# szpiech/garlic

Hardware: AMD Instinct MI355X
Metric: LOD-windows/sec (SNPs x inds / winsize) (higher is better)
Workload: dtype f64

## Files before the change

### garlic_amd/csrc/garlic_hip.hip

```cpp
#include "../../include/garlic_hip.h"
#include "lod_kernels.hpp"
#include "variant_kernels.hpp"
#include "ld_kernels.hpp"
#include "ld_multi_kernel.hpp"
#include "tgls_ring_kernel.hpp"
#include "tgls_feed_kernel.hpp"
#include "tgls_feed_multi_kernel.hpp"
#include "wlod_strip_kernel.hpp"
#include "wlod_small_kernel.hpp"
#include "coverage_kernel.hpp"
#include "roh_segments_kernel.hpp"
#include "feed_kernel.hpp"
#include "wlod_feed_kernel.hpp"

#include <algorithm>
#include <chrono>
#include <functional>
#include <memory>
#include <mutex>
#include <queue>
#include <cmath>
#include <cstdarg>
#include <cstdio>
#include <cstdlib>
// ... 2267 lines not shown
        hipError_t e = hipSuccess;
        if (where == GARLIC_HOST) {
            if ((rc = stage.reserve((size_t)(rows * ld)))) { stage.release(); return rc; }
            e = hipMemcpyAsync(stage.p, src, (size_t)(rows * ld), hipMemcpyHostToDevice, s);
            src = stage.p;
        }
        if (e == hipSuccess) {
            const int64_t waves = rows * nblk;
            hipLaunchKernelGGL(phase_planes_kernel, dim3((unsigned)((waves + 3) / 4)), dim3(256), 0, s, src,
                               ld, locus_begin + done, rows, p->nind, nblk, p->nloci, p->d_phase.p);
            e = hipGetLastError();
        }
        if (e == hipSuccess) e = hipStreamSynchronize(s);
        if (e != hipSuccess) { stage.release(); return fail(GARLIC_ERR_HIP, "set_phase: %s", hipGetErrorString(e)); }
    }
    stage.release();
    p->have_phase = true;
    return GARLIC_OK;
}

static int reserve_skew_buf(garlic_panel *p, DevBuf<double> &buf, int32_t winsize, bool zero)
{
    int rc;
    const size_t nskew = SKEW_FRONT + ((size_t)p->nloci + winsize + 64) * winsize;
    if ((rc = buf.reserve(nskew))) return rc;
    if (zero) {
        HIP_TRY(hipMemsetAsync(buf.p, 0, sizeof(double) * nskew, p->ctx->stream));
    } else {
        HIP_TRY(hipMemsetAsync(buf.p, 0, sizeof(double) * SKEW_FRONT, p->ctx->stream));
        const size_t body = SKEW_FRONT + (size_t)p->nloci * winsize;
        HIP_TRY(hipMemsetAsync(buf.p + body, 0, sizeof(double) * (nskew - body), p->ctx->stream));
    }
    return GARLIC_OK;
}
static int reserve_skew(garlic_panel *p, int32_t winsize, bool zero = true)
{
    return reserve_skew_buf(p, p->d_skew, winsize, zero);
}

static void drop_ld_sets(garlic_panel *p) { p->ld_sets.clear(); }
static bool select_ld(garlic_panel *p, int32_t winsize)
{
    if (p->have_ld && p->ld_winsize == winsize) return true;
    for (size_t i = 0; i < p->ld_sets.size(); i++) {
        garlic_panel::LdSet &set = *p->ld_sets[i];
        if (set.W != winsize) continue;
        std::swap(set.skew.p, p->d_skew.p);
        std::swap(set.skew.cap, p->d_skew.cap);
        std::swap(set.group, p->ld_group);
        if (p->have_ld) set.W = p->ld_winsize;
        else p->ld_sets.erase(p->ld_sets.begin() + (ptrdiff_t)i);
        p->ld_winsize = winsize;
        p->have_ld = true;
        p->rld_valid = false;
        return true;
    }
    return false;
}
static void stash_ld(garlic_panel *p, int32_t group)
{
    if (!p->have_ld) return;
    std::unique_ptr<garlic_panel::LdSet> set(new garlic_panel::LdSet);
    set->W = p->ld_winsize;
    set->group = group;
    std::swap(set->skew.p, p->d_skew.p);
    std::swap(set->skew.cap, p->d_skew.cap);
    p->ld_sets.push_back(std::move(set));
    p->have_ld = false;
    p->rld_valid = false;
    p->ld_winsize = 0;
    p->ld_group = -1;
}
static void drop_all_ld(garlic_panel *p)
{
    drop_ld_sets(p);
    p->d_skew.release();
    p->d_rld.release();
    p->have_ld = p->rld_valid = false;
    p->ld_winsize = 0;
    p->ld_group = -1;
}

static int install_ld(garlic_panel *p, int32_t winsize, const double *src, bool skew_done = false)
{
    int rc;
    hipStream_t s = p->ctx->stream;
    if (!skew_done) {
        if ((rc = reserve_skew(p, winsize))) return rc;
        for (int c = 0; c < p->nchr; c++)
            hipLaunchKernelGGL(skew_reciprocal_kernel, dim3(1024), dim3(256), 0, s, src,
                               p->d_skew.p + SKEW_FRONT, p->chr_off[c], p->chr_off[c + 1], winsize);
    }
    HIP_TRY(hipGetLastError());
    HIP_TRY(hipStreamSynchronize(s));
    p->d_rld.release();
    p->rld_valid = false;
    p->have_ld = true;
    p->ld_winsize = winsize;
    p->ld_group = -1;
    if (!p->ld_multi_active) {
        drop_ld_sets(p);
        p->ld_pair_passes = p->ld_sum_passes = 0;
    }
    return GARLIC_OK;
}

static int ensure_rld(garlic_panel *p)
{
    if (p->rld_valid) return GARLIC_OK;
    int rc;
    const int32_t W = p->ld_winsize;
    if ((rc = p->d_rld.reserve((size_t)p->nloci * W))) return rc;
    for (int c = 0; c < p->nchr; c++)
        hipLaunchKernelGGL(unskew_kernel, dim3(1024), dim3(256), 0, p->ctx->stream, p->d_skew.p + SKEW_FRONT, p->d_rld.p,
                           p->chr_off[c], p->chr_off[c + 1], W);
    HIP_TRY(hipGetLastError());
    p->rld_valid = true;
    return GARLIC_OK;
}

int garlic_panel_set_ld(garlic_panel *p, int32_t winsize, const double *ld, int32_t where)
{
    if (!p || !ld) return fail(GARLIC_ERR_INVALID, "panel and ld are required");
    if (winsize <= 1) return fail(GARLIC_ERR_INVALID, "winsize must be > 1");
    int rc;
    if ((rc = set_device(p->ctx))) return rc;
    const size_t n = (size_t)p->nloci * winsize;
    const double *src = ld;
    if (where == GARLIC_HOST) {
        if ((rc = p->d_stage64.reserve(n))) return rc;
        HIP_TRY(hipMemcpyAsync(p->d_stage64.p, ld, sizeof(double) * n, hipMemcpyHostToDevice,
                               p->ctx->stream));
        src = p->d_stage64.p;
    }
    rc = install_ld(p, winsize, src);
    p->d_stage64.release();
    return rc;
}

static bool ld_pairs_on_mfma(int32_t winsize, int32_t phased)
{
    const int mfma_nj = 1 + (30 + winsize) / 32;
    const bool pair_flat = getenv("GARLIC_LD_PAIR_FLAT") && winsize <= 32;
    return !phased && !pair_flat && winsize > LD_SMALL_MAX_W && mfma_nj <= 5 && !getenv("GARLIC_LD_PAIR_NO_MFMA") &&
           !getenv("GARLIC_LD_PAIR_TILED") && !getenv("GARLIC_LD_PAIR_L2");
}
static bool ld_sums_by_snp(int32_t winsize)
{
    const int col_threads = (winsize + 16 + WAVE - 1) / WAVE * WAVE;
    return winsize > LD_COL_B && winsize <= 512 && col_threads <= LD_COL_MAX_THREADS && !getenv("GARLIC_LD_SUM_BY_COLUMN") &&
           !getenv("GARLIC_LD_SUM_L2");
}

static int ld_check(garlic_panel *p, int32_t winsize, int32_t phased)
{
    if (!p) return fail(GARLIC_ERR_INVALID, "panel is NULL");
    if (!p->have_geno) return fail(GARLIC_ERR_STATE, "panel needs genotypes before LD weights");
    if (phased && !p->have_phase)
        return fail(GARLIC_ERR_STATE, "phased LD weights need garlic_panel_set_phase first");
    if (phased && !p->have_freq)
        return fail(GARLIC_ERR_STATE, "phased LD weights need the allele frequencies (garlic_panel_set_freq)");
    if (winsize <= 1) return fail(GARLIC_ERR_INVALID, "winsize must be > 1");
    if ((int64_t)p->nloci * winsize * 2 >= ((int64_t)1 << 40))
        return fail(GARLIC_ERR_INVALID, "LD table of %lld x %d too large", (long long)p->nloci, winsize);
    return set_device(p->ctx);
}

int garlic_ld_counts(garlic_panel *p, int32_t winsize, int32_t phased, const int32_t *sub_idx, int32_t n_sub,
                     int32_t *locus_counts, int32_t *pair_counts, int32_t where)
{
    int rc;
    if ((rc = ld_check(p, winsize, phased))) return rc;
    if (!locus_counts || !pair_counts) return fail(GARLIC_ERR_INVALID, "count buffers are required");
    if (n_sub < 0 || (n_sub > 0 && !sub_idx)) return fail(GARLIC_ERR_INVALID, "bad LD subsample");
    hipStream_t s = p->ctx->stream;
    const int nblk = (int)(p->nind_pad / WAVE);
    std::vector<uint64_t> sub((size_t)nblk, 0);
    if (!sub_idx) {
        for (int i = 0; i < p->nind; i++) sub[i >> 6] |= (uint64_t)1 << (i & 63);
    } else {
        for (int k = 0; k < n_sub; k++) {
            const int i = sub_idx[k];
            if (i < 0 || i >= p->nind)
                return fail(GARLIC_ERR_INVALID, "LD subsample index %d outside panel of %d", i, p->nind);
            if (sub[i >> 6] & ((uint64_t)1 << (i & 63)))
                return fail(GARLIC_ERR_INVALID, "LD subsample index %d given twice", i);
            sub[i >> 6] |= (uint64_t)1 << (i & 63);
        }
    }
    DevBuf<uint64_t> &d_sub = p->lds.sub, &d_m = p->lds.m, &d_h = p->lds.h, &d_o = p->lds.o;
    DevBuf<int32_t> &d_loc = p->lds.loc, &d_pair = p->lds.pair;
    const size_t npl = (size_t)nblk * p->nloci, npair = (size_t)p->nloci * winsize * 2;
    if ((rc = d_sub.reserve(nblk)) || (rc = d_m.reserve(npl)) || (rc = d_h.reserve(npl))) return rc;
    if (phased && (rc = d_o.reserve(npl))) return rc;
    int32_t *loc = locus_counts, *pair = pair_counts;
    if (where == GARLIC_HOST) {
        if ((rc = d_loc.reserve((size_t)p->nloci * 2)) || (rc = d_pair.reserve(npair))) return rc;
        loc = d_loc.p; pair = d_pair.p;
    }
    const bool pair_flat = getenv("GARLIC_LD_PAIR_FLAT") && winsize <= 32;
    const int lane_stage = std::min(nblk, getenv("GARLIC_LD_LANE_STAGE") ? atoi(getenv("GARLIC_LD_LANE_STAGE")) : 4);
    const int lane_dc = winsize - 1 <= 16 ? 16 : 32;
    const size_t lane_lds = sizeof(uint64_t) * (phased ? 4 : 2) * (size_t)lane_stage * (LD_LANE_T + winsize - 1);
    const int mfma_nj = 1 + (30 + winsize) / 32;
    const bool pair_mfma = ld_pairs_on_mfma(winsize, phased);
    const bool fuse_hr2 = p->lds.fuse_request && pair_mfma && ld_sums_by_snp(winsize);
    if (p->lds.fuse_request && !fuse_hr2) {
        p->lds.fuse_request = false;
        return fail(GARLIC_ERR_STATE, "internal: LD fusion requested for a shape the pair kernel does not take");
    }
    p->lds.fuse_request = false;
    p->lds.fused_done = false;
    const bool pair_lane = !pair_mfma && !pair_flat && winsize - 1 <= 256 && lane_lds <= 150 * 1024 && !getenv("GARLIC_LD_PAIR_TILED") &&
                           !getenv("GARLIC_LD_PAIR_L2");
    const bool pair_tiled = !pair_mfma && !pair_flat && !pair_lane && winsize - 1 <= 256 && !getenv("GARLIC_LD_PAIR_L2");
    hipError_t e = hipMemcpyAsync(d_sub.p, sub.data(), sizeof(uint64_t) * nblk, hipMemcpyHostToDevice, s);
    if (e == hipSuccess && !pair_tiled && !pair_flat && !pair_lane && !pair_mfma) e = hipMemsetAsync(pair, 0, sizeof(int32_t) * npair, s);
    if (e != hipSuccess) return fail(GARLIC_ERR_HIP, "LD counts: %s", hipGetErrorString(e));
    uint64_t planes_key = 0xCBF29CE484222325ull;
    for (uint64_t w : sub) planes_key = (planes_key ^ w) * 0x100000001B3ull;
    planes_key = (planes_key ^ (uint64_t)(phased ? 2 : 1)) * 0x100000001B3ull;
    planes_key = (planes_key ^ p->geno_epoch) * 0x100000001B3ull;
    planes_key = (planes_key ^ (uint64_t)nblk) * 0x100000001B3ull;
    if ((rc = p->lds.loc_planes.reserve((size_t)p->nloci * 2))) return rc;
    if (!(p->lds.planes_valid && p->lds.planes_key == planes_key) || getenv("GARLIC_LD_NO_PLANE_CACHE")) {
        p->lds.planes_valid = false;
        if (phased)
            hipLaunchKernelGGL(ld_planes_kernel<true>, dim3((unsigned)p->nwordrows), dim3(256), 0, s, p->d_packed.p,
                               p->nwordrows, nblk, d_sub.p, p->nloci, d_m.p, d_h.p, d_o.p, p->lds.loc_planes.p);
        else
            hipLaunchKernelGGL(ld_planes_kernel<false>, dim3((unsigned)p->nwordrows), dim3(256), 0, s, p->d_packed.p,
                               p->nwordrows, nblk, d_sub.p, p->nloci, d_m.p, d_h.p, (uint64_t *)nullptr, p->lds.loc_planes.p);
        e = hipGetLastError();
        if (e != hipSuccess) return fail(GARLIC_ERR_HIP, "LD planes: %s", hipGetErrorString(e));
        p->lds.planes_key = planes_key;
        p->lds.planes_valid = true;
    }
    e = hipMemcpyAsync(loc, p->lds.loc_planes.p, sizeof(int32_t) * p->nloci * 2, hipMemcpyDeviceToDevice, s);
    if (e != hipSuccess) return fail(GARLIC_ERR_HIP, "LD counts: %s", hipGetErrorString(e));
    const int pair_threads = (winsize - 1 + WAVE - 1) / WAVE * WAVE;
    const size_t pair_lds = sizeof(uint64_t) * (phased ? 4 : 2) * LD_PAIR_BLK * (LD_PAIR_T + winsize - 1);
    if (pair_tiled && pair_lds > 48 * 1024) {
        const void *fn = phased ? (const void *)ld_pair_tiled_kernel<true> : (const void *)ld_pair_tiled_kernel<false>;
        hipError_t ae = hipFuncSetAttribute(fn, hipFuncAttributeMaxDynamicSharedMemorySize, (int)pair_lds);
        if (ae != hipSuccess) return fail(GARLIC_ERR_HIP, "LD counts: %s", hipGetErrorString(ae));
    }
    if (pair_tiled) {
        std::vector<LdPairChr> pc;
        int64_t blocks = 0;
        for (int c = 0; c < p->nchr; c++) {
            pc.push_back(LdPairChr{p->chr_off[c], p->chr_off[c + 1], blocks});
            blocks += (p->chr_nloci[c] + LD_PAIR_T - 1) / LD_PAIR_T;
        }
        DevBuf<LdPairChr> &d_pc = p->lds.pair_chrs;
        if ((rc = d_pc.reserve(pc.size()))) return rc;
        e = hipMemcpyAsync(d_pc.p, pc.data(), sizeof(LdPairChr) * pc.size(), hipMemcpyHostToDevice, s);
        if (e != hipSuccess) return fail(GARLIC_ERR_HIP, "LD counts: %s", hipGetErrorString(e));
        if (phased)
            hipLaunchKernelGGL(ld_pair_tiled_kernel<true>, dim3((unsigned)blocks), dim3(pair_threads), pair_lds, s, d_m.p,
                               d_h.p, d_o.p, p->d_phase.p, nblk, p->nloci, d_pc.p, p->nchr, winsize, pair);
        else
            hipLaunchKernelGGL(ld_pair_tiled_kernel<false>, dim3((unsigned)blocks), dim3(pair_threads), pair_lds, s, d_m.p,
                               d_h.p, (const uint64_t *)nullptr, (const uint64_t *)nullptr, nblk, p->nloci, d_pc.p,
                               p->nchr, winsize, pair);
        e = hipGetLastError();
        if (e == hipSuccess) e = hipStreamSynchronize(s);
        if (e != hipSuccess) return fail(GARLIC_ERR_HIP, "LD counts: %s", hipGetErrorString(e));
    }
    if (pair_mfma) {
        std::vector<LdPairChr> pc;
        int64_t blocks = 0;
        for (int c = 0; c < p->nchr; c++) {
            pc.push_back(LdPairChr{p->chr_off[c], p->chr_off[c + 1], blocks});
            blocks += (p->chr_nloci[c] + LDM_TI - 1) / LDM_TI;
        }
        DevBuf<LdPairChr> &d_pc = p->lds.pair_chrs;
        if ((rc = d_pc.reserve(pc.size()))) return rc;
        e = hipMemcpyAsync(d_pc.p, pc.data(), sizeof(LdPairChr) * pc.size(), hipMemcpyHostToDevice, s);
        const void *fn = fuse_hr2 ? (mfma_nj <= 2 ? (const void *)ld_pair_mfma_kernel<2, true> : mfma_nj == 3 ? (const void *)ld_pair_mfma_kernel<3, true>
                                     : mfma_nj == 4 ? (const void *)ld_pair_mfma_kernel<4, true> : (const void *)ld_pair_mfma_kernel<5, true>)
                                  : (mfma_nj <= 2 ? (const void *)ld_pair_mfma_kernel<2, false> : mfma_nj == 3 ? (const void *)ld_pair_mfma_kernel<3, false>
                                     : mfma_nj == 4 ? (const void *)ld_pair_mfma_kernel<4, false> : (const void *)ld_pair_mfma_kernel<5, false>);
        const int nj = std::max(2, mfma_nj);
        const size_t lds = std::max((size_t)2 * 2 * (4 + nj - 1) * WAVE * 16, fuse_hr2 ? LDM_XT_BYTES : (size_t)0);
        const double *a_hf = nullptr;
        double *a_c = nullptr;
        if (fuse_hr2) {
            const size_t n = (size_t)p->nloci * winsize;
            if ((rc = p->lds.hf.reserve(p->nloci)) || (rc = p->lds.fwd.reserve(2 * n + 256))) return rc;
            hipLaunchKernelGGL(ld_homfreq_kernel, dim3((unsigned)((p->nloci + 255) / 256)), dim3(256), 0, s, p->lds.loc_planes.p, p->nloci,
                               p->lds.hf.p);
            a_hf = p->lds.hf.p;
            a_c = p->lds.fwd.p;
        }
        if (e == hipSuccess && lds > 48 * 1024) e = hipFuncSetAttribute(fn, hipFuncAttributeMaxDynamicSharedMemorySize, (int)lds);
        if (e != hipSuccess) return fail(GARLIC_ERR_HIP, "LD counts: %s", hipGetErrorString(e));
        const uint64_t *a_m = d_m.p, *a_h = d_h.p;
        const LdPairChr *a_pc = d_pc.p;
        int a_nblk = nblk, a_nchr = p->nchr, a_w = winsize;
        int64_t a_nloci = p->nloci;
        void *kargs[] = {(void *)&a_m, (void *)&a_h, (void *)&a_nblk, (void *)&a_nloci, (void *)&a_pc, (void *)&a_nchr, (void *)&a_w, (void *)&pair,
                         (void *)&a_hf, (void *)&a_c};
        e = hipLaunchKernel(fn, dim3((unsigned)blocks), dim3(256), kargs, lds, s);
        if (e == hipSuccess) e = hipStreamSynchronize(s);
        if (e != hipSuccess) return fail(GARLIC_ERR_HIP, "LD counts: %s", hipGetErrorString(e));
        p->lds.fused_done = fuse_hr2;
    }
    if (pair_lane) {
        std::vector<LdPairChr> pc;
        int64_t blocks = 0;
        for (int c = 0; c < p->nchr; c++) {
            pc.push_back(LdPairChr{p->chr_off[c], p->chr_off[c + 1], blocks});
            blocks += (p->chr_nloci[c] + LD_LANE_T - 1) / LD_LANE_T;
        }
        DevBuf<LdPairChr> &d_pc = p->lds.pair_chrs;
        if ((rc = d_pc.reserve(pc.size()))) return rc;
        e = hipMemcpyAsync(d_pc.p, pc.data(), sizeof(LdPairChr) * pc.size(), hipMemcpyHostToDevice, s);
        const void *fn = lane_dc == 16 ? (phased ? (const void *)ld_pair_lane_kernel<true, 16> : (const void *)ld_pair_lane_kernel<false, 16>)
                                       : (phased ? (const void *)ld_pair_lane_kernel<true, 32> : (const void *)ld_pair_lane_kernel<false, 32>);
        if (e == hipSuccess && lane_lds > 48 * 1024) e = hipFuncSetAttribute(fn, hipFuncAttributeMaxDynamicSharedMemorySize, (int)lane_lds);
        if (e != hipSuccess) return fail(GARLIC_ERR_HIP, "LD counts: %s", hipGetErrorString(e));
        const uint64_t *a_m = d_m.p, *a_h = d_h.p, *a_o = phased ? d_o.p : nullptr, *a_f = phased ? p->d_phase.p : nullptr;
        const LdPairChr *a_pc = d_pc.p;
        int a_nblk = nblk, a_nchr = p->nchr, a_w = winsize, a_stage = lane_stage;
        int64_t a_nloci = p->nloci;
        void *kargs[] = {(void *)&a_m, (void *)&a_h, (void *)&a_o, (void *)&a_f, (void *)&a_nblk, (void *)&a_nloci, (void *)&a_pc,
                         (void *)&a_nchr, (void *)&a_w, (void *)&a_stage, (void *)&pair};
        e = hipLaunchKernel(fn, dim3((unsigned)blocks), dim3(LD_LANE_T), kargs, lane_lds, s);
        if (e == hipSuccess) e = hipStreamSynchronize(s);
        if (e != hipSuccess) return fail(GARLIC_ERR_HIP, "LD counts: %s", hipGetErrorString(e));
    }
    if (pair_flat) {
        const unsigned grid = (unsigned)(((int64_t)p->nloci * winsize + 255) / 256);
        if (phased)
            hipLaunchKernelGGL(ld_pair_flat_kernel<true>, dim3(grid), dim3(256), 0, s, d_m.p, d_h.p, d_o.p, p->d_phase.p, nblk,
                               p->nloci, p->d_chr_off.p, p->nchr, winsize, pair);
        else
            hipLaunchKernelGGL(ld_pair_flat_kernel<false>, dim3(grid), dim3(256), 0, s, d_m.p, d_h.p, (const uint64_t *)nullptr,
                               (const uint64_t *)nullptr, nblk, p->nloci, p->d_chr_off.p, p->nchr, winsize, pair);
    }
    for (int c = 0; !pair_tiled && !pair_flat && !pair_lane && !pair_mfma && c < p->nchr; c++) {
        if (phased)
            hipLaunchKernelGGL(ld_pair_phased_kernel, dim3((unsigned)p->chr_nloci[c]), dim3(256), 0, s, d_m.p,
                               d_h.p, d_o.p, p->d_phase.p, nblk, p->nloci, p->chr_off[c], p->chr_off[c + 1],
                               winsize, pair);
        else
            hipLaunchKernelGGL(ld_pair_kernel, dim3((unsigned)p->chr_nloci[c]), dim3(256), 0, s, d_m.p, d_h.p,
                               nblk, p->nloci, p->chr_off[c], p->chr_off[c + 1], winsize, pair);
    }
    e = hipGetLastError();
    if (e == hipSuccess && where == GARLIC_HOST) {
        e = hipMemcpyAsync(locus_counts, loc, sizeof(int32_t) * p->nloci * 2, hipMemcpyDeviceToHost, s);
        if (e == hipSuccess)
            e = hipMemcpyAsync(pair_counts, pair, sizeof(int32_t) * npair, hipMemcpyDeviceToHost, s);
    }
    if (e == hipSuccess) e = hipStreamSynchronize(s);
    if (e != hipSuccess) return fail(GARLIC_ERR_HIP, "LD counts: %s", hipGetErrorString(e));
    return GARLIC_OK;
}

int garlic_ld_finish(garlic_panel *p, int32_t winsize, int32_t phased, const int32_t *locus_counts,
                     const int32_t *pair_counts, double *ld_out, int32_t where)
{
    int rc;
    if ((rc = ld_check(p, winsize, phased))) return rc;
    if (!locus_counts || !pair_counts) return fail(GARLIC_ERR_INVALID, "count buffers are required");
    hipStream_t s = p->ctx->stream;
    const size_t n = (size_t)p->nloci * winsize;
    DevBuf<int32_t> &d_loc = p->lds.loc, &d_pair = p->lds.pair;
    DevBuf<double> &d_hf = p->lds.hf, &d_fwd = p->lds.fwd, &d_bwd = p->lds.bwd, &d_ld = p->lds.ld;
    DevBuf<LdSumChr> &d_sum_chrs = p->lds.sum_chrs;
    const int32_t *loc = locus_counts, *pair = pair_counts;
    hipError_t e = hipSuccess;
    if (where == GARLIC_HOST) {
        if ((rc = d_loc.reserve((size_t)p->nloci * 2)) || (rc = d_pair.reserve(n * 2))) return rc;
        e = hipMemcpyAsync(d_loc.p, locus_counts, sizeof(int32_t) * p->nloci * 2, hipMemcpyHostToDevice, s);
        if (e == hipSuccess)
            e = hipMemcpyAsync(d_pair.p, pair_counts, sizeof(int32_t) * n * 2, hipMemcpyHostToDevice, s);
        loc = d_loc.p; pair = d_pair.p;
    }
    if (winsize <= LD_SMALL_MAX_W && !getenv("GARLIC_LD_NO_FLAT")) {
        if ((rc = d_hf.reserve(p->nloci))) return rc;
        double *ld = ld_out;
        if (where == GARLIC_HOST || !ld_out) {
            if ((rc = d_ld.reserve(n))) return rc;
            ld = d_ld.p;
        }
        if (e == hipSuccess) e = hipMemsetAsync(ld, 0, sizeof(double) * n, s);
        if (e == hipSuccess && phased) e = hipMemcpyAsync(d_hf.p, p->freq.data(), sizeof(double) * p->nloci, hipMemcpyHostToDevice, s);
        if (e != hipSuccess) return fail(GARLIC_ERR_HIP, "LD finish: %s", hipGetErrorString(e));
        if (!phased)
            hipLaunchKernelGGL(ld_homfreq_kernel, dim3((unsigned)((p->nloci + 255) / 256)), dim3(256), 0, s, loc, p->nloci, d_hf.p);
        garlic_ctx *ctx = p->ctx;
        const int slot = (int)(ctx->n_calls % garlic_ctx::HIST);
        (void)hipEventRecord(ctx->hist0[slot], s);
        hipLaunchKernelGGL(ld_sum_flat_kernel, dim3((unsigned)((n + 255) / 256)), dim3(256), 0, s, pair, d_hf.p, p->d_chr_off.p,
                           p->nchr, p->nloci, winsize, ld);
        (void)hipEventRecord(ctx->hist1[slot], s);
        ctx->n_calls++;
        e = hipGetLastError();
        if (e != hipSuccess) return fail(GARLIC_ERR_HIP, "LD finish: %s", hipGetErrorString(e));
        if ((rc = install_ld(p, winsize, ld, false))) return rc;
        if (where == GARLIC_HOST && ld_out) {
            e = hipMemcpyAsync(ld_out, ld, sizeof(double) * n, hipMemcpyDeviceToHost, s);
            if (e == hipSuccess) e = hipStreamSynchronize(s);
            if (e != hipSuccess) return fail(GARLIC_ERR_HIP, "LD finish: %s", hipGetErrorString(e));
        }
        return GARLIC_OK;
    }
    const int col_threads = (winsize + 16 + WAVE - 1) / WAVE * WAVE;
    const bool by_snp = ld_sums_by_snp(winsize);
    const bool have_table = p->lds.fused_done && by_snp;
    p->lds.fused_done = false;
    const bool tiled = by_snp || (winsize <= LD_SUM_MAX_W && !getenv("GARLIC_LD_SUM_L2"));
    const int sum_b = by_snp ? std::min(LD_COL_B, col_threads - winsize) : LD_SUM_B;
    if ((rc = d_hf.reserve(p->nloci)) || (rc = d_fwd.reserve(by_snp ? 2 * n + 256 : n)) || (!by_snp && (rc = d_bwd.reserve(n))))
        return rc;
    double *ld = ld_out;
    const bool weights_only = by_snp && !ld_out;
    if (!weights_only && (where == GARLIC_HOST || !ld_out)) {
        if ((rc = d_ld.reserve(n))) return rc;
        ld = d_ld.p;
    }
    if (weights_only) {
    } else if (by_snp) {
        for (int c = 0; c < p->nchr && e == hipSuccess; c++) {
            const int64_t lo = p->chr_off[c], hi = p->chr_off[c + 1], from = std::max(lo, hi - winsize + 1);
            if (hi > from) e = hipMemsetAsync(ld + from * winsize, 0, sizeof(double) * (size_t)(hi - from) * winsize, s);
        }
    } else {
        e = hipMemsetAsync(ld, 0, sizeof(double) * n, s);
    }
    if (e != hipSuccess) return fail(GARLIC_ERR_HIP, "LD finish: %s", hipGetErrorString(e));
    if (phased) {
        e = hipMemcpyAsync(d_hf.p, p->freq.data(), sizeof(double) * p->nloci, hipMemcpyHostToDevice, s);
        if (e != hipSuccess) return fail(GARLIC_ERR_HIP, "LD finish: %s", hipGetErrorString(e));
    } else {
        hipLaunchKernelGGL(ld_homfreq_kernel, dim3((unsigned)((p->nloci + 255) / 256)), dim3(256), 0, s, loc,
                           p->nloci, d_hf.p);
    }
    std::vector<LdSumChr> sum_chrs;
    int64_t sum_blocks = 0;
    for (int c = 0; tiled && c < p->nchr; c++) {
        const int64_t nstarts = p->chr_off[c + 1] - p->chr_off[c] - winsize + 1;
        if (nstarts < 1) continue;
        sum_chrs.push_back(LdSumChr{p->chr_off[c], nstarts, sum_blocks});
        sum_blocks += (nstarts + sum_b - 1) / sum_b;
    }
    if (tiled && (rc = d_sum_chrs.reserve(std::max<size_t>(sum_chrs.size(), 1)))) return rc;
    if (by_snp && (rc = reserve_skew(p, winsize, false))) return rc;
    for (int c = 0; c < p->nchr; c++) {
        const int64_t lo = p->chr_off[c], hi = p->chr_off[c + 1];
        const size_t hr2_lds = sizeof(double) * (LD_HR2_T + winsize + (size_t)LD_HR2_T * (winsize + 1));
        if (have_table)
            ;
        else if (by_snp && hr2_lds <= 64 * 1024 && !getenv("GARLIC_LD_HR2_PLAIN"))
            hipLaunchKernelGGL(ld_hr2_tile_kernel, dim3((unsigned)((hi - lo + LD_HR2_T - 1) / LD_HR2_T)), dim3(256),
                               hr2_lds, s, pair, d_hf.p, lo, hi, winsize, d_fwd.p);
        else if (by_snp)
            hipLaunchKernelGGL(ld_hr2_kernel<true>, dim3((unsigned)(hi - lo)), dim3(128), 0, s, pair, d_hf.p, lo, hi,
                               winsize, d_fwd.p, (double *)nullptr);
        else
            hipLaunchKernelGGL(ld_hr2_kernel<false>, dim3((unsigned)(hi - lo)), dim3(256), 0, s, pair, d_hf.p, lo, hi,
                               winsize, d_fwd.p, d_bwd.p);
        if (hi - lo >= winsize && !tiled)
            hipLaunchKernelGGL(ld_sum_kernel, dim3((unsigned)(hi - lo - winsize + 1)), dim3(256), 0, s, d_fwd.p, d_bwd.p,
                               lo, winsize, ld);
    }
    if (tiled && !sum_chrs.empty()) {
        e = hipMemcpyAsync(d_sum_chrs.p, sum_chrs.data(), sizeof(LdSumChr) * sum_chrs.size(), hipMemcpyHostToDevice, s);
        if (e != hipSuccess) return fail(GARLIC_ERR_HIP, "LD finish: %s", hipGetErrorString(e));
        const int threads = by_snp ? col_threads : (winsize + WAVE - 1) / WAVE * WAVE;
        const int col_pieces = (threads * 8 + 1023) / 1024;
        const size_t lds = by_snp ? sizeof(double) * std::max<size_t>((size_t)LD_COL_BATCH * LD_COL_NBATCH * col_pieces * 128 + 130, (size_t)threads * 17)
                                  : sizeof(double) * 2 * (2 * (size_t)winsize - 1 + 128 + threads);
        garlic_ctx *ctx = p->ctx;
        const int slot = (int)(ctx->n_calls % garlic_ctx::HIST);
        (void)hipEventRecord(ctx->hist0[slot], s);
        if (by_snp) {
            static_assert(LD_COL_MAX_THREADS <= 128 * LD_COL_MAX_PIECES, "one instantiation per request count");
            const void *fn = col_pieces == 1 ? (const void *)ld_sum_col_kernel<1> : col_pieces == 2 ? (const void *)ld_sum_col_kernel<2>
                           : col_pieces == 3 ? (const void *)ld_sum_col_kernel<3> : col_pieces == 4 ? (const void *)ld_sum_col_kernel<4>
                                                                                                    : (const void *)ld_sum_col_kernel<5>;
            if (lds > 48 * 1024) {
                e = hipFuncSetAttribute(fn, hipFuncAttributeMaxDynamicSharedMemorySize, (int)lds);
                if (e != hipSuccess) return fail(GARLIC_ERR_HIP, "LD finish: %s", hipGetErrorString(e));
            }
            const double *a_c = d_fwd.p;
            const LdSumChr *a_chrs = d_sum_chrs.p;
            int a_nchr = (int)sum_chrs.size(), a_w = winsize, a_b = sum_b;
            double *a_ld = ld, *a_d = p->d_skew.p + SKEW_FRONT;
            unsigned a_nwork = (unsigned)sum_blocks;
            void *kargs[] = {(void *)&a_c, (void *)&a_chrs, (void *)&a_nchr, (void *)&a_w, (void *)&a_b, (void *)&a_ld, (void *)&a_d, (void *)&a_nwork};
            e = hipLaunchKernel(fn, dim3((a_nwork + 7u) / 8u * 8u), dim3(threads), kargs, lds, s);
            if (e != hipSuccess) return fail(GARLIC_ERR_HIP, "LD finish: %s", hipGetErrorString(e));
        }
        else
            hipLaunchKernelGGL(ld_sum_tiled_kernel, dim3((unsigned)sum_blocks), dim3(threads), lds, s, d_fwd.p, d_bwd.p,
                               d_sum_chrs.p, (int)sum_chrs.size(), winsize, ld);
        (void)hipEventRecord(ctx->hist1[slot], s);
        ctx->n_calls++;
    }
    e = hipGetLastError();
    if (e != hipSuccess) return fail(GARLIC_ERR_HIP, "LD finish: %s", hipGetErrorString(e));
    if ((rc = install_ld(p, winsize, ld, by_snp))) return rc;
    if (where == GARLIC_HOST && ld_out) {
        e = hipMemcpyAsync(ld_out, ld, sizeof(double) * n, hipMemcpyDeviceToHost, s);
        if (e == hipSuccess) e = hipStreamSynchronize(s);
        if (e != hipSuccess) return fail(GARLIC_ERR_HIP, "LD finish: %s", hipGetErrorString(e));
    }
    return GARLIC_OK;
}

int garlic_panel_compute_ld(garlic_panel *p, int32_t winsize, int32_t phased, const int32_t *sub_idx,
                            int32_t n_sub, double *ld_out, int32_t where)
{
    int rc;
    if ((rc = ld_check(p, winsize, phased))) return rc;
    DevBuf<int32_t> &d_loc = p->lds.loc, &d_pair = p->lds.pair;
    const bool fuse = ld_pairs_on_mfma(winsize, phased) && ld_sums_by_snp(winsize) && !getenv("GARLIC_LD_UNFUSED");
    if ((rc = d_loc.reserve((size_t)p->nloci * 2)) || (rc = d_pair.reserve(fuse ? 2 : (size_t)p->nloci * winsize * 2)))
        return rc;
    p->lds.fuse_request = fuse;
    if ((rc = garlic_ld_counts(p, winsize, phased, sub_idx, n_sub, d_loc.p, d_pair.p, GARLIC_DEVICE))) {
        p->lds.fuse_request = false;
        return rc;
    }
    if (where == GARLIC_DEVICE || !ld_out)
        return garlic_ld_finish(p, winsize, phased, d_loc.p, d_pair.p, ld_out, GARLIC_DEVICE);
    DevBuf<double> &d_ld = p->lds.ld;
    if ((rc = d_ld.reserve((size_t)p->nloci * winsize))) return rc;
    rc = garlic_ld_finish(p, winsize, phased, d_loc.p, d_pair.p, d_ld.p, GARLIC_DEVICE);
    if (rc == GARLIC_OK) {
        hipError_t e = hipMemcpy(ld_out, d_ld.p, sizeof(double) * p->nloci * winsize, hipMemcpyDeviceToHost);
        if (e != hipSuccess) rc = fail(GARLIC_ERR_HIP, "LD copy-out: %s", hipGetErrorString(e));
    }
    return rc;
}

static int ld_col_threads(int32_t winsize) { return (winsize + 16 + WAVE - 1) / WAVE * WAVE; }

struct LdMultiPlan {
    std::vector<int32_t> uniq;
    std::vector<std::vector<int32_t>> groups;
    size_t n_shared = 0;
    int32_t wtab = 0;
};
static LdMultiPlan ld_multi_plan(const int32_t *winsizes, int32_t n_sizes)
{
    LdMultiPlan plan;
    plan.uniq.assign(winsizes, winsizes + n_sizes);
    std::sort(plan.uniq.begin(), plan.uniq.end());
    plan.uniq.erase(std::unique(plan.uniq.begin(), plan.uniq.end()), plan.uniq.end());
    const char *solo_env = getenv("GARLIC_LD_MULTI_SOLO");
    const bool solo = solo_env && atoi(solo_env) != 0;
    std::vector<int32_t> sharing, alone;
    for (int32_t w : plan.uniq) (!solo && ld_sums_by_snp(w) ? sharing : alone).push_back(w);
    if (sharing.size() < 2) {
        alone = plan.uniq;
        sharing.clear();
    }
    for (int32_t w : sharing) {
        const bool fits = !plan.groups.empty() && plan.groups.back().size() < (size_t)LDM_MAX_SIZES &&
                          ldms_lds_bytes(ld_col_threads(w), (int)plan.groups.back().size()) <= LDMS_LDS_MAX;
        if (!fits) plan.groups.emplace_back();
        plan.groups.back().push_back(w);
    }
    plan.n_shared = plan.groups.size();
    plan.wtab = sharing.empty() ? 0 : sharing.back();
    for (int32_t w : alone) plan.groups.push_back(std::vector<int32_t>{w});
    return plan;
}

typedef std::vector<std::unique_ptr<garlic_panel::LdSet>> LdSetPool;
static std::unique_ptr<garlic_panel::LdSet> ld_pool_take(LdSetPool &pool, int32_t winsize)
{
    for (size_t i = 0; i < pool.size(); i++)
        if (pool[i]->W == winsize) {
            std::unique_ptr<garlic_panel::LdSet> set = std::move(pool[i]);
            pool.erase(pool.begin() + (ptrdiff_t)i);
            return set;
        }
    std::unique_ptr<garlic_panel::LdSet> set(new garlic_panel::LdSet);
    set->W = winsize;
    return set;
}

static int ld_build_table(garlic_panel *p, int32_t W, int32_t phased, const int32_t *loc, const int32_t *pair)
{
    int rc;
    hipStream_t s = p->ctx->stream;
    const size_t n = (size_t)p->nloci * W;
    if ((rc = p->lds.hf.reserve(p->nloci)) || (rc = p->lds.fwd.reserve(2 * n + 256))) return rc;
    if (phased)
        HIP_TRY(hipMemcpyAsync(p->lds.hf.p, p->freq.data(), sizeof(double) * p->nloci, hipMemcpyHostToDevice, s));
    else
        hipLaunchKernelGGL(ld_homfreq_kernel, dim3((unsigned)((p->nloci + 255) / 256)), dim3(256), 0, s, loc, p->nloci, p->lds.hf.p);
    const size_t hr2_lds = sizeof(double) * (LD_HR2_T + W + (size_t)LD_HR2_T * (W + 1));
    for (int c = 0; c < p->nchr; c++) {
        const int64_t lo = p->chr_off[c], hi = p->chr_off[c + 1];
        if (hr2_lds <= 64 * 1024 && !getenv("GARLIC_LD_HR2_PLAIN"))
            hipLaunchKernelGGL(ld_hr2_tile_kernel, dim3((unsigned)((hi - lo + LD_HR2_T - 1) / LD_HR2_T)), dim3(256), hr2_lds, s, pair,
                               p->lds.hf.p, lo, hi, W, p->lds.fwd.p);
        else
            hipLaunchKernelGGL(ld_hr2_kernel<true>, dim3((unsigned)(hi - lo)), dim3(128), 0, s, pair, p->lds.hf.p, lo, hi, W,
                               p->lds.fwd.p, (double *)nullptr);
    }
    HIP_TRY(hipGetLastError());
    return GARLIC_OK;
}

static int ld_multi_group(garlic_panel *p, const std::vector<int32_t> &g, int32_t gid, int32_t wtab, double *const *dev_ld,
                          LdSetPool &pool)
{
    int rc;
    hipStream_t s = p->ctx->stream;
    const int32_t W = g.back(), wmin = g.front();
    const int threads = ld_col_threads(W), B = std::min(LD_COL_B, threads - W), pieces = (threads * 8 + 1023) / 1024;
    const size_t lds = ldms_lds_bytes(threads, (int)g.size() - 1);
    std::vector<LdMultiChr> chrs;
    int64_t blocks = 0;
    for (int c = 0; c < p->nchr; c++) {
        const int64_t lo = p->chr_off[c], hi = p->chr_off[c + 1], nstarts = hi - lo - wmin + 1;
        if (nstarts < 1) continue;
        chrs.push_back(LdMultiChr{lo, hi, nstarts, blocks});
        blocks += (nstarts + B - 1) / B;
    }
    std::vector<std::unique_ptr<garlic_panel::LdSet>> sets;
    LdMultiSmall small{};
    small.n = (int32_t)g.size() - 1;
    for (size_t i = 0; i < g.size(); i++) {
        sets.push_back(ld_pool_take(pool, g[i]));
// ... 1457 lines not shown
```

### garlic_amd/csrc/ld_kernels.hpp

```cpp
#pragma once
#include "lod_kernels.hpp"
#include "tgls_math.hpp"
#include "variant_kernels.hpp"

namespace garlic {

__device__ __forceinline__ double x86_nan_if_nan(double v)
{
    return v != v ? f64_from_bits(X86_DEFAULT_NAN) : v;
}

__device__ __forceinline__ uint32_t ld_writelane(uint32_t v, int lane, uint32_t old)
{
    asm("v_writelane_b32 %0, %1, %2" : "+v"(old) : "s"(v), "n"(lane));
    return old;
}

template <bool PHASED>
__global__ void __launch_bounds__(256)
ld_planes_kernel(const uint32_t *__restrict__ packed, int64_t nwordrows, int nblk,
                 const uint64_t *__restrict__ submask, int64_t nloci, uint64_t *__restrict__ planeM,
                 uint64_t *__restrict__ planeH, uint64_t *__restrict__ planeO, int32_t *__restrict__ counts)
{
    __shared__ int32_t red[4][16][2];
// ... 566 lines not shown
        LD_COL_WAIT_CASE(57)
        LD_COL_WAIT_CASE(58)
        LD_COL_WAIT_CASE(59)
        LD_COL_WAIT_CASE(60)
        LD_COL_WAIT_CASE(61)
        LD_COL_WAIT_CASE(62)
        LD_COL_WAIT_CASE(63)
#undef LD_COL_WAIT_CASE
    default: asm volatile("s_waitcnt vmcnt(0)" ::: "memory"); break;
    }
}

#define LD_COL_ADD(q) "v_add_f64 %[a" #q "], %[a" #q "], %[h]\n\t"
#define LD_COL_OPS(a)                                                                                              \
    [a0] "+v"(a[0]), [a1] "+v"(a[1]), [a2] "+v"(a[2]), [a3] "+v"(a[3]), [a4] "+v"(a[4]), [a5] "+v"(a[5]),          \
    [a6] "+v"(a[6]), [a7] "+v"(a[7]), [a8] "+v"(a[8]), [a9] "+v"(a[9]), [a10] "+v"(a[10]), [a11] "+v"(a[11]),      \
    [a12] "+v"(a[12]), [a13] "+v"(a[13]), [a14] "+v"(a[14]), [a15] "+v"(a[15]), [a16] "+v"(a[16]),                 \
    [a17] "+v"(a[17]), [a18] "+v"(a[18]), [a19] "+v"(a[19]), [a20] "+v"(a[20]), [a21] "+v"(a[21]),                 \
    [a22] "+v"(a[22]), [a23] "+v"(a[23]), [a24] "+v"(a[24]), [a25] "+v"(a[25]), [a26] "+v"(a[26]),                 \
    [a27] "+v"(a[27]), [a28] "+v"(a[28]), [a29] "+v"(a[29]), [a30] "+v"(a[30]), [a31] "+v"(a[31])
#define LD_COL_JUMP "s_getpc_b64 s[98:99]\n\ts_add_u32 s98, s98, %[off]\n\ts_addc_u32 s99, s99, 0\n\ts_setpc_b64 s[98:99]\n\t"
__device__ __forceinline__ void ld_col_adds(double (&a)[LD_COL_B], double h, bool ascending, int first)
{
    static_assert(LD_COL_B == 32, "32 adds are written out");
    const uint32_t off = (uint32_t)__builtin_amdgcn_readfirstlane(first * 8 + (ascending ? 12 + 32 * 8 + 4 : 12));
    asm volatile(LD_COL_JUMP
                 LD_COL_ADD(31) LD_COL_ADD(30) LD_COL_ADD(29) LD_COL_ADD(28) LD_COL_ADD(27) LD_COL_ADD(26)
                 LD_COL_ADD(25) LD_COL_ADD(24) LD_COL_ADD(23) LD_COL_ADD(22) LD_COL_ADD(21) LD_COL_ADD(20)
                 LD_COL_ADD(19) LD_COL_ADD(18) LD_COL_ADD(17) LD_COL_ADD(16) LD_COL_ADD(15) LD_COL_ADD(14)
                 LD_COL_ADD(13) LD_COL_ADD(12) LD_COL_ADD(11) LD_COL_ADD(10) LD_COL_ADD(9) LD_COL_ADD(8) LD_COL_ADD(7)
                 LD_COL_ADD(6) LD_COL_ADD(5) LD_COL_ADD(4) LD_COL_ADD(3) LD_COL_ADD(2) LD_COL_ADD(1) LD_COL_ADD(0)
                 "s_branch LD_COL_END_%=\n\t"
                 LD_COL_ADD(0) LD_COL_ADD(1) LD_COL_ADD(2) LD_COL_ADD(3) LD_COL_ADD(4) LD_COL_ADD(5)
                 LD_COL_ADD(6) LD_COL_ADD(7) LD_COL_ADD(8) LD_COL_ADD(9) LD_COL_ADD(10) LD_COL_ADD(11) LD_COL_ADD(12)
                 LD_COL_ADD(13) LD_COL_ADD(14) LD_COL_ADD(15) LD_COL_ADD(16) LD_COL_ADD(17) LD_COL_ADD(18)
                 LD_COL_ADD(19) LD_COL_ADD(20) LD_COL_ADD(21) LD_COL_ADD(22) LD_COL_ADD(23) LD_COL_ADD(24)
                 LD_COL_ADD(25) LD_COL_ADD(26) LD_COL_ADD(27) LD_COL_ADD(28) LD_COL_ADD(29) LD_COL_ADD(30)
                 LD_COL_ADD(31)
                 "LD_COL_END_%=:\n\t"
                 : LD_COL_OPS(a) : [h] "v"(h), [off] "s"(off) : "s98", "s99", "scc");
}
template <int PIECES>
__global__ void __launch_bounds__(LD_COL_MAX_THREADS)
ld_sum_col_kernel(const double *__restrict__ C, const LdSumChr *__restrict__ chrs, int nchr, int W, int B,
                  double *__restrict__ ld, double *__restrict__ D, unsigned nwork)
{
    const unsigned per_xcd = gridDim.x >> 3;
    const unsigned vblock = (blockIdx.x & 7u) * per_xcd + (blockIdx.x >> 3);
    if (vblock >= nwork) return;
    constexpr int BATCH = LD_COL_BATCH, NB = LD_COL_NBATCH, NRING = BATCH * NB, STEADY = (NB - 2) * BATCH * PIECES;
    static_assert(STEADY <= 63, "requests that can be counted");
    extern __shared__ double ld_rows[];
    const int tl = threadIdx.x, P = 2 * W;
    const int wave = __builtin_amdgcn_readfirstlane(threadIdx.x >> 6);
    int c = 0;
    while (c + 1 < nchr && (int64_t)vblock >= chrs[c + 1].block0) c++;
    const int64_t s0 = chrs[c].lo + ((int64_t)vblock - chrs[c].block0) * B;
    const int ns = (int)min<int64_t>(B, chrs[c].lo + chrs[c].nstarts - s0);
    const int nsteps = ns + W - 1, nbatches = (nsteps + BATCH - 1) / BATCH;
    const uint32_t ring = (uint32_t)(uintptr_t)(__attribute__((address_space(3))) double *)ld_rows;
    constexpr uint32_t row_bytes = (uint32_t)PIECES * 1024u, ring_bytes = row_bytes * NRING;
    const uint32_t lane16 = (uint32_t)(tl & 63) * 16u;
    const char *req_row = reinterpret_cast<const char *>(C + s0 * P);
    int req_e = W - 1, req_left = nsteps;
    uint32_t req_off = 0;
    auto request_batch = [&]() {
#pragma unroll
        for (int u = 0; u < BATCH; u++) {
            if (req_left > 0) {
                const char *g = req_row + (int64_t)(req_e & ~1) * 8;
#pragma unroll
                for (int q = 0; q < PIECES; q++)
                    asm volatile("s_mov_b32 m0, %0\n\ts_nop 0\n\tglobal_load_lds_dwordx4 %1, %2"
                                 :: "s"(ring + req_off + (uint32_t)q * 1024u), "v"(lane16), "s"(g + q * 1024) : "memory");
                req_row += (int64_t)P * 8;
                req_e--;
                req_left--;
            }
            req_off += row_bytes;
        }
        if (req_off == ring_bytes) req_off = 0;
    };
    if (wave == 0)
        for (int k = 0; k < NB - 1; k++) request_batch();
    double acc[LD_COL_B];
#pragma unroll
    for (int q = 0; q < LD_COL_B; q++) acc[q] = 0.0;
    uint32_t rd_addr = ring + (uint32_t)tl * 8u;
    const uint32_t rd_end = rd_addr + ring_bytes;
    uint32_t odd = (uint32_t)(W - 1) & 1u;
    static_assert(BATCH % 2 == 0, "the parity of W-1-j repeats per batch");
    for (int k = 0; k < nbatches; k++) {
        if (wave == 0) {
            const int rows_later = min(nsteps, (k + NB - 1) * BATCH) - (k + 1) * BATCH;
            if (rows_later == (NB - 2) * BATCH) asm volatile("s_waitcnt vmcnt(%0)" ::"n"(STEADY) : "memory");
            else ld_col_wait(max(rows_later, 0) * PIECES);
        }
        __syncthreads();
        if (wave == 0) request_batch();
        const int j0 = k * BATCH;
        double h[BATCH];
#pragma unroll
        for (int u = 0; u < BATCH; u++)
            asm volatile("ds_read_b64 %0, %1" : "=v"(h[u]) : "v"(rd_addr + (uint32_t)u * row_bytes + ((odd ^ (uint32_t)(u & 1)) * 8u)) : "memory");
        asm volatile("s_waitcnt lgkmcnt(0)" ::: "memory");
        rd_addr += BATCH * row_bytes;
        if (rd_addr == rd_end) rd_addr -= ring_bytes;
#pragma unroll
        for (int u = 0; u < BATCH; u++) {
            const int j = j0 + u;
#ifdef GARLIC_LDS_ABL_NO_ADDS
            if (j < nsteps && h[u] == 1.2345e-300) {
#else
            if (j < nsteps) {
#endif
                const bool leaving = j >= W;
                ld_col_adds(acc, h[u], leaving,
                            leaving ? j - W + 1 : (j < LD_COL_B - 1 ? LD_COL_B - 1 - j : 0));
            }
        }
    }
#ifndef GARLIC_LDS_ABL_NO_LD
    if (ld) {
#pragma unroll
        for (int q = 0; q < LD_COL_B; q++) {
            const int k = tl - q;
            if (q < ns && k >= 0 && k < W) ld[(s0 + q) * W + k] = x86_nan_if_nan(acc[q]);
        }
    }
#else
    if (acc[0] == 1.2345e-300) ld[s0 * W + tl] = acc[1] + acc[2] + acc[3] + acc[31] + acc[16];
#endif
#ifdef GARLIC_LDS_ABL_NO_D
    if (acc[5] != 1.2345e-300) return;
#endif
    if (!D) return;
    __syncthreads();
    double *tile = ld_rows;
    const int nthreads = blockDim.x;
    for (int q0 = 0; q0 < LD_COL_B; q0 += 16) {
#pragma unroll
        for (int u = 0; u < 16; u++)
            if (q0 == 0) tile[tl * 17 + u] = reciprocal_x86(x86_nan_if_nan(acc[u]));
            else tile[tl * 17 + u] = reciprocal_x86(x86_nan_if_nan(acc[16 + u]));
        __syncthreads();
        for (int e = tl; e < nthreads * 16; e += nthreads) {
            const int t2 = e >> 4, u = e & 15, q = q0 + u, k = t2 - q;
            if (q < ns && k >= 0 && k < W) D[(s0 + t2) * W + k] = tile[t2 * 17 + u];
        }
        __syncthreads();
    }
}

}

namespace garlic {

constexpr int LDM_TI = 128;
typedef int ldm_i32x4 __attribute__((ext_vector_type(4)));

typedef int ldm_i32x8 __attribute__((ext_vector_type(8)));
typedef float ldm_f32x16 __attribute__((ext_vector_type(16)));

__device__ __forceinline__ uint32_t ldm_spread8(uint32_t x)
{
    uint32_t t = (x | (x << 12)) & 0x000F000Fu;
    t = (t | (t << 6)) & 0x03030303u;
    return (t | (t << 3)) & 0x11111111u;
}

constexpr int LDM_XT = 33;
constexpr size_t LDM_XT_BYTES = ((size_t)4 * 32 * LDM_XT + 256) * 8;

template <int NJ, bool HR2>
__global__ void __launch_bounds__(256, 2)
ld_pair_mfma_kernel(const uint64_t *__restrict__ planeM, const uint64_t *__restrict__ planeH, int nblk, int64_t nloci,
                    const LdPairChr *__restrict__ chrs, int nchr, int W, int32_t *__restrict__ pair,
                    const double *__restrict__ hf, double *__restrict__ C)
{
    constexpr int NT = 4 + NJ - 1;
    static_assert(NT * 32 <= 256, "one staged SNP per thread");
    constexpr int BUF = 2 * NT * WAVE * 16;
    extern __shared__ __attribute__((aligned(16))) unsigned char ldm_lds[];
    const int tid = threadIdx.x, lane = tid & 63;
    const int wave = __builtin_amdgcn_readfirstlane(tid >> 6);
    int c = 0;
    while (c + 1 < nchr && (int64_t)blockIdx.x >= chrs[c + 1].block0) c++;
    const int64_t hi = chrs[c].hi;
    const int64_t i0 = chrs[c].lo + ((int64_t)blockIdx.x - chrs[c].block0) * LDM_TI;
    const bool mine = tid < NT * 32;
    const bool in = mine && i0 + tid < hi;
    uint64_t wm = 0, wh = 0;
    auto fetch = [&](int b) {
        const int64_t g = (int64_t)b * nloci + i0 + (in ? tid : 0);
        wm = in ? planeM[g] : 0;
        wh = in ? planeH[g] : 0;
    };
    auto stage = [&](int buf) {
        if (!mine) return;
        const int tile = tid >> 5, r = tid & 31;
#pragma unroll
        for (int pl = 0; pl < 2; pl++) {
            const uint64_t w = pl ? wh : wm;
#pragma unroll
            for (int h = 0; h < 2; h++) {
                const uint32_t x = (uint32_t)(w >> (32 * h));
                unsigned char *dst = ldm_lds + buf * BUF + (((pl * NT + tile) * WAVE) + h * 32 + r) * 16;
                *reinterpret_cast<uint4 *>(dst) = make_uint4(ldm_spread8(x & 0xFFu), ldm_spread8((x >> 8) & 0xFFu),
                                                             ldm_spread8((x >> 16) & 0xFFu), ldm_spread8(x >> 24));
            }
        }
    };
    ldm_f32x16 acc[NJ][2];
#pragma unroll
    for (int q = 0; q < NJ; q++)
#pragma unroll
        for (int pl = 0; pl < 2; pl++)
#pragma unroll
            for (int k = 0; k < 16; k++) acc[q][pl][k] = 0.0f;
    fetch(0);
    stage(0);
    if (nblk > 1) fetch(1);
    __syncthreads();
    const int one = 0x7F7F7F7F;
    for (int b = 0; b < nblk; b++) {
        const int buf = b & 1;
#ifndef GARLIC_LDM_ABL_NO_STAGE
        if (b + 1 < nblk) stage(buf ^ 1);
#endif
        if (b + 2 < nblk) fetch(b + 2);
#pragma unroll
        for (int pl = 0; pl < 2; pl++) {
            ldm_i32x8 fb[NJ];
#pragma unroll
            for (int q = 0; q < NJ; q++) {
                const ldm_i32x4 f = *reinterpret_cast<const ldm_i32x4 *>(ldm_lds + buf * BUF + (((pl * NT + wave + q) * WAVE) + lane) * 16);
                fb[q] = ldm_i32x8{f[0], f[1], f[2], f[3], 0, 0, 0, 0};
            }
#pragma unroll
            for (int q = 0; q < NJ; q++)
                acc[q][pl] = __builtin_amdgcn_mfma_scale_f32_32x32x64_f8f6f4(fb[0], fb[q], acc[q][pl], 4, 4, 0, one, 0, one);
        }
        __syncthreads();
    }
    const int col = lane & 31, rh = 4 * (lane >> 5);
    const int64_t it = i0 + wave * 32;
    if (HR2) {
        double *xt = reinterpret_cast<double *>(ldm_lds) + (size_t)wave * 32 * LDM_XT;
        double *hfs = reinterpret_cast<double *>(ldm_lds) + (size_t)4 * 32 * LDM_XT;
        if (mine) hfs[tid] = in ? hf[i0 + tid] : 0.0;
        __syncthreads();
        const int P = 2 * W;
#pragma unroll
        for (int q = 0; q < NJ; q++) {
            const int64_t j = it + q * 32 + col;
            const double HB = hfs[wave * 32 + q * 32 + col];
            const bool okB = HB > 0 && HB < 1;
            const double pB = HB * (1 - HB);
#pragma unroll
            for (int k = 0; k < 16; k++) {
                const int base = (k & 3) + 8 * (k >> 2);
                if (32 * q + 31 - base < 0 || 32 * q - (base + 4) >= W) continue;
                const int il = base + rh;
                const int64_t i = it + il;
                const int64_t d = j - i;
                const double HA = hfs[wave * 32 + il];
                double f = 0.0, b = 0.0;
                if (HA > 0 && HA < 1 && okB) {
                    double HAB = (double)(int)(acc[q][1][k] * 4.0f);
                    HAB /= (double)(int)(acc[q][0][k] * 4.0f);
                    const double H = HAB - HA * HB, HH = H * H;
                    const double vf = HH / (HA * (1 - HA) * HB * (1 - HB));
                    const double vb = HH / (pB * HA * (1 - HA));
                    f = (vf > 1) ? 1.0 : x86_nan_if_nan(vf);
                    b = (vb > 1) ? 1.0 : x86_nan_if_nan(vb);
                }
                if (i < hi && j < hi && d >= 0 && d < W) C[i * P + W - 1 + d] = d == 0 ? 1.0 : f;
                xt[col * LDM_XT + il] = b;
                __builtin_amdgcn_sched_barrier(0);
            }
            __builtin_amdgcn_fence(__ATOMIC_ACQ_REL, "wavefront");
#pragma unroll 4
            for (int r = 0; r < 16; r++) {
                const int jl = 2 * r + (lane >> 5);
                const int64_t jj = it + q * 32 + jl, ii = it + col;
                const int64_t d = jj - ii;
                const double v = xt[jl * LDM_XT + col];
                if (ii < hi && jj < hi && d >= 1 && d < W) C[jj * P + W - 1 - d] = v;
            }
            __builtin_amdgcn_fence(__ATOMIC_ACQ_REL, "wavefront");
        }
        return;
    }
#pragma unroll
    for (int q = 0; q < NJ; q++) {
        const int64_t j = it + q * 32 + col;
#pragma unroll
        for (int k = 0; k < 16; k++) {
            const int64_t i = it + (k & 3) + 8 * (k >> 2) + rh;
            const int64_t d = j - i;
            if (i < hi && d >= 0 && d < W) {
                int2 v = make_int2((int)(acc[q][0][k] * 4.0f), (int)(acc[q][1][k] * 4.0f));
                if (d == 0) v = make_int2(0, 0);
#ifdef GARLIC_LDM_ABL_NO_STORE
                if (v.x != 0x7FFFFFF1) continue;
#endif
// ... 8 lines not shown
```

Before: 7.193 billion.

## Add streaming LD column-sum kernel with async global-to-LDS ring buffer

Adds ld_sum_stream_kernel, which gives each block a span of K column batches. A dedicated loader wave streams the forward LD rows into an LDS ring buffer using global_load_lds_dwordx4 while G teams of threads consume successive batches in turn. The intent is to reuse overlapping window rows across adjacent batches within a block instead of reloading them per batch, and to overlap global loads with the accumulation. It also writes the reciprocal table through per-wave LDS tiles using only wave barriers. The cost is more complex scheduling, large LDS use, fewer blocks, and possible load imbalance depending on the span heuristic.

```diff
diff --git a/garlic_amd/csrc/garlic_hip.hip b/garlic_amd/csrc/garlic_hip.hip
--- a/garlic_amd/csrc/garlic_hip.hip
+++ b/garlic_amd/csrc/garlic_hip.hip
@@ -2443,6 +2443,33 @@
            !getenv("GARLIC_LD_SUM_L2");
 }
 
+struct LdStreamPlan {
+    bool ok;
+    int T, B, G, K, threads, loader_wave;
+    size_t lds;
+};
+static LdStreamPlan ld_sum_stream_plan(int32_t winsize, int64_t nloci)
+{
+    LdStreamPlan pl{};
+    if (!ld_sums_by_snp(winsize) || getenv("GARLIC_LD_SUM_NO_STREAM")) return pl;
+    pl.T = (winsize + 16 + WAVE - 1) / WAVE * WAVE;
+    pl.B = std::min(LD_COL_B, pl.T - winsize);
+    pl.G = (pl.B + winsize - 1 + pl.B - 1) / pl.B;
+    pl.lds = ld_stream_lds_bytes(winsize, pl.T);
+    if (pl.G * pl.T > LD_STREAM_MAX_THREADS || pl.lds > LD_STREAM_LDS_MAX) return pl;
+    const bool own_wave = pl.G * pl.T + WAVE <= LD_STREAM_MAX_THREADS;
+    pl.threads = pl.G * pl.T + (own_wave ? WAVE : 0);
+    pl.loader_wave = own_wave ? pl.G * pl.T / WAVE : 0;
+    int k = (int)std::ceil((winsize - 1) / (0.055 * pl.B));
+    const int64_t even = nloci / pl.B / 2048;
+    if (even < k) k = (int)std::max<int64_t>(even, pl.G);
+    if (const char *v = getenv("GARLIC_LD_STREAM_SPAN")) k = atoi(v);
+    else k = (k + pl.G - 1) / pl.G * pl.G;
+    pl.K = std::min(std::max(k, 1), LD_STREAM_MAX_SPAN);
+    pl.ok = true;
+    return pl;
+}
+
 static int ld_check(garlic_panel *p, int32_t winsize, int32_t phased)
 {
     if (!p) return fail(GARLIC_ERR_INVALID, "panel is NULL");
@@ -2730,13 +2757,15 @@
         hipLaunchKernelGGL(ld_homfreq_kernel, dim3((unsigned)((p->nloci + 255) / 256)), dim3(256), 0, s, loc,
                            p->nloci, d_hf.p);
     }
+    const LdStreamPlan stream = by_snp ? ld_sum_stream_plan(winsize, p->nloci) : LdStreamPlan{};
+    const int64_t sum_unit = stream.ok ? (int64_t)stream.K * sum_b : sum_b;
     std::vector<LdSumChr> sum_chrs;
     int64_t sum_blocks = 0;
     for (int c = 0; tiled && c < p->nchr; c++) {
         const int64_t nstarts = p->chr_off[c + 1] - p->chr_off[c] - winsize + 1;
         if (nstarts < 1) continue;
         sum_chrs.push_back(LdSumChr{p->chr_off[c], nstarts, sum_blocks});
-        sum_blocks += (nstarts + sum_b - 1) / sum_b;
+        sum_blocks += (nstarts + sum_unit - 1) / sum_unit;
     }
     if (tiled && (rc = d_sum_chrs.reserve(std::max<size_t>(sum_chrs.size(), 1)))) return rc;
     if (by_snp && (rc = reserve_skew(p, winsize, false))) return rc;
@@ -2768,7 +2797,18 @@
         garlic_ctx *ctx = p->ctx;
         const int slot = (int)(ctx->n_calls % garlic_ctx::HIST);
         (void)hipEventRecord(ctx->hist0[slot], s);
-        if (by_snp) {
+        if (stream.ok) {
+            const void *fn = (const void *)ld_sum_stream_kernel;
+            if (stream.lds > 48 * 1024) {
+                e = hipFuncSetAttribute(fn, hipFuncAttributeMaxDynamicSharedMemorySize, (int)stream.lds);
+                if (e != hipSuccess) return fail(GARLIC_ERR_HIP, "LD finish: %s", hipGetErrorString(e));
+            }
+            const unsigned nwork = (unsigned)sum_blocks;
+            hipLaunchKernelGGL(ld_sum_stream_kernel, dim3((nwork + 7u) / 8u * 8u), dim3((unsigned)stream.threads), stream.lds, s,
+                               (const double *)d_fwd.p, (const LdSumChr *)d_sum_chrs.p, (int)sum_chrs.size(), (int)winsize, stream.B,
+                               stream.G, stream.T, stream.K, stream.loader_wave, ld, p->d_skew.p + SKEW_FRONT, nwork);
+        }
+        else if (by_snp) {
             static_assert(LD_COL_MAX_THREADS <= 128 * LD_COL_MAX_PIECES, "one instantiation per request count");
             const void *fn = col_pieces == 1 ? (const void *)ld_sum_col_kernel<1> : col_pieces == 2 ? (const void *)ld_sum_col_kernel<2>
                            : col_pieces == 3 ? (const void *)ld_sum_col_kernel<3> : col_pieces == 4 ? (const void *)ld_sum_col_kernel<4>
diff --git a/garlic_amd/csrc/ld_kernels.hpp b/garlic_amd/csrc/ld_kernels.hpp
--- a/garlic_amd/csrc/ld_kernels.hpp
+++ b/garlic_amd/csrc/ld_kernels.hpp
@@ -742,6 +742,139 @@
     }
 }
 
+constexpr int LD_STREAM_BATCH = 4;
+constexpr int LD_STREAM_NB = 4;
+constexpr int LD_STREAM_MAX_THREADS = 1024;
+constexpr size_t LD_STREAM_LDS_MAX = 128 * 1024;
+constexpr int LD_STREAM_MAX_SPAN = 4096;
+__host__ __device__ inline uint32_t ld_stream_ring_bytes(int W)
+{
+    const uint32_t need = (uint32_t)LD_STREAM_NB * LD_STREAM_BATCH * 16u * (uint32_t)W + 2048u;
+    uint32_t r = 4096;
+    while (r < need) r <<= 1;
+    return r;
+}
+__host__ __device__ inline size_t ld_stream_lds_bytes(int W, int T) { return (size_t)ld_stream_ring_bytes(W) + (size_t)2 * (T / 64) * 64 * 17 * sizeof(double); }
+
+__global__ void __launch_bounds__(LD_STREAM_MAX_THREADS) __attribute__((amdgpu_waves_per_eu(6)))
+ld_sum_stream_kernel(const double *__restrict__ C, const LdSumChr *__restrict__ chrs, int nchr, int W, int B, int G, int T, int K,
+                     int loader_wave, double *__restrict__ ld, double *__restrict__ D, unsigned nwork)
+{
+    const unsigned per_xcd = gridDim.x >> 3;
+    const unsigned vblock = (blockIdx.x & 7u) * per_xcd + (blockIdx.x >> 3);
+    if (vblock >= nwork) return;
+    constexpr int BATCH = LD_STREAM_BATCH, NB = LD_STREAM_NB;
+    extern __shared__ double ld_rows[];
+    const int wave = __builtin_amdgcn_readfirstlane(threadIdx.x >> 6);
+    const int team = wave / (T >> 6);
+    const int tl = (int)threadIdx.x - team * T, lane = tl & 63;
+    int c = 0;
+    while (c + 1 < nchr && (int64_t)vblock >= chrs[c + 1].block0) c++;
+    const int64_t first = ((int64_t)vblock - chrs[c].block0) * K * B;
+    const int64_t span_s0 = chrs[c].lo + first;
+    const int span_ns = (int)min<int64_t>((int64_t)K * B, chrs[c].nstarts - first);
+    const int nrows = span_ns + W - 1, nbat = (span_ns + B - 1) / B, niter = (nrows + BATCH - 1) / BATCH;
+    const uint32_t ring = (uint32_t)(uintptr_t)(__attribute__((address_space(3))) double *)ld_rows;
+    const uint32_t ring_bytes = ld_stream_ring_bytes(W), mask = ring_bytes - 1u;
+    double *tiles = ld_rows + (ring_bytes >> 3);
+    const int batch_bytes = BATCH * 16 * W;
+    const int total_chunks = (nrows * 16 * W + 1023) >> 10;
+    const char *src = reinterpret_cast<const char *>(C + span_s0 * (int64_t)(2 * W));
+    const uint32_t lane16 = (uint32_t)(threadIdx.x & 63) * 16u;
+    int issued = 0;
+    auto request_to = [&](int target) {
+        for (; issued < target; issued++)
+            asm volatile("s_mov_b32 m0, %0\n\ts_nop 0\n\tglobal_load_lds_dwordx4 %1, %2"
+                         :: "s"(ring + (((uint32_t)issued << 10) & mask)), "v"(lane16), "s"(src + ((int64_t)issued << 10)) : "memory");
+    };
+    if (wave == loader_wave) request_to(min(total_chunks, ((NB - 1) * batch_bytes + 1023) >> 10));
+    double acc[LD_COL_B];
+#pragma unroll
+    for (int q = 0; q < LD_COL_B; q++) acc[q] = 0.0;
+    int b = team, jbase = -team * B, ns = 0, nsteps = 0;
+    int64_t s0 = 0;
+    auto enter = [&]() {
+        if (team < G && b < nbat) {
+            s0 = span_s0 + (int64_t)b * B;
+            ns = min(B, span_ns - b * B);
+            nsteps = ns + W - 1;
+        } else {
+            ns = 0;
+            nsteps = 0;
+        }
+    };
+    enter();
+    const uint32_t rowstep = (uint32_t)(2 * W - 1) * 8u;
+    uint32_t rd = ((uint32_t)(W - 1 + tl + team * B) * 8u) & mask;
+    double h[BATCH];
+    auto read_rows = [&](uint32_t at) {
+#pragma unroll
+        for (int u = 0; u < BATCH; u++)
+            asm volatile("ds_read_b64 %0, %1" : "=v"(h[u]) : "v"(ring + ((at + (uint32_t)u * rowstep) & mask)) : "memory");
+        asm volatile("s_waitcnt lgkmcnt(0)" ::: "memory");
+    };
+    auto add_rows = [&]() {
+#pragma unroll
+        for (int u = 0; u < BATCH; u++) {
+            const int j = jbase + u;
+            if (j >= 0 && j < nsteps) {
+                const bool leaving = j >= W;
+                ld_col_adds(acc, h[u], leaving,
+                            leaving ? j - W + 1 : (j < LD_COL_B - 1 ? LD_COL_B - 1 - j : 0));
+            }
+        }
+    };
+    for (int k = 0; k < niter; k++) {
+        if (wave == loader_wave) {
+            const int needed = min(total_chunks, ((k + 1) * batch_bytes + 1023) >> 10);
+            ld_col_wait(issued - needed);
+        }
+        __syncthreads();
+        if (wave == loader_wave) request_to(min(total_chunks, ((k + NB) * batch_bytes + 1023) >> 10));
+        read_rows(rd);
+        rd = (rd + BATCH * rowstep) & mask;
+        add_rows();
+        const int fin = nsteps - 1 - jbase;
+        if (__builtin_expect(nsteps > 0 && fin >= 0 && fin < BATCH, 0)) {
+            if (ld) {
+#pragma unroll
+                for (int q = 0; q < LD_COL_B; q++) {
+                    const int kk = tl - q;
+                    if (q < ns && kk >= 0 && kk < W) ld[(s0 + q) * W + kk] = x86_nan_if_nan(acc[q]);
+                }
+            }
+            if (D) {
+                double *tile = tiles + (size_t)((b & 1) * (T >> 6) + (tl >> 6)) * (64 * 17);
+                const int tbase = tl & ~63;
+#pragma unroll
+                for (int q0 = 0; q0 < LD_COL_B; q0 += 16) {
+#pragma unroll
+                    for (int u = 0; u < 16; u++) tile[lane * 17 + u] = reciprocal_x86(x86_nan_if_nan(acc[q0 + u]));
+                    __builtin_amdgcn_fence(__ATOMIC_RELEASE, "wavefront");
+                    __builtin_amdgcn_wave_barrier();
+                    for (int e = lane; e < 64 * 16; e += 64) {
+                        const int t2l = e >> 4, u = e & 15, q = q0 + u, t2 = tbase + t2l, kk = t2 - q;
+                        if (q < ns && kk >= 0 && kk < W) D[(s0 + t2) * W + kk] = tile[t2l * 17 + u];
+                    }
+                    __builtin_amdgcn_fence(__ATOMIC_RELEASE, "wavefront");
+                    __builtin_amdgcn_wave_barrier();
+                }
+            }
+#pragma unroll
+            for (int q = 0; q < LD_COL_B; q++) acc[q] = 0.0;
+            b += G;
+            jbase -= G * B;
+            rd = (rd + (uint32_t)(G * B) * 8u) & mask;
+            enter();
+            if (jbase + BATCH > 0 && nsteps > 0) {
+                read_rows(rd - BATCH * rowstep);
+                add_rows();
+            }
+        }
+        jbase += BATCH;
+    }
+}
+
 }
 
 namespace garlic {
```

Result: no change. 7.194 billion, median of 3 (+0.0%).
